# resero-labs/latok

Measured on NVIDIA B200. Metric: tokenized_text_throughput, higher is better.
Workload: dtype u8

## Files before the change

### latok_b200/csrc/latok_capi.cu

```cuda
#include "../../include/latok_b200.h"
#include "latok_internal.h"
#include "_gen/latok_tables.h"

#include <cstdarg>
#include <cstdio>
#include <cstdlib>
#include <cstring>
#include <new>
#include <vector>

using namespace latok;

namespace {

thread_local char g_err[512] = "";

int fail(int code, const char *fmt, ...)
{
    va_list ap;
    va_start(ap, fmt);
    vsnprintf(g_err, sizeof g_err, fmt, ap);
    va_end(ap);
    return code;
}
// ... 72 lines not shown
{
    if (na != nb) return false;
    std::vector<uint32_t> x(a, a + na), y(b, b + nb);
    for (auto v : x) {
        bool found = false;
        for (auto &w : y) if (w == v) { w = 0xFFFFFFFFu; found = true; break; }
        if (!found) return false;
    }
    return true;
}

}

struct Batch {
    DevBuf<uint8_t> d_in;
    DevBuf<long long> d_off, d_first, d_char_off, d_tok_off;
    DevBuf<int8_t> d_splits, d_feats, d_matrix;
    DevBuf<int32_t> d_spans;
    DevBuf<uint32_t> d_spans16;
    DevBuf<Result> d_result;
    PinBuf<Result> h_result;
    PinBuf<uint8_t> h_in;
    PinBuf<long long> h_off;
    cudaEvent_t ev_h2d = nullptr;
    cudaEvent_t ev_index = nullptr;
    cudaEvent_t ev_k0 = nullptr, ev_k1 = nullptr;
    cudaEvent_t ev_kdone = nullptr;
    bool submitted = false, sized = false, inputs_on_stream = false;
    const uint8_t *cur_in = nullptr;
    const long long *cur_off = nullptr;
    long long n_strings = 0, n_bytes = 0;
    uint32_t what = 0;
    long long n_chars = 0, n_tokens = 0, walks = 0;
    float kernel_ms = 0.f;
    void release()
    {
        d_in.release(); d_off.release(); d_first.release(); d_char_off.release(); d_tok_off.release();
        d_splits.release(); d_feats.release(); d_matrix.release(); d_spans.release(); d_spans16.release();
        d_result.release(); h_result.release(); h_in.release(); h_off.release();
        for (cudaEvent_t *ev : {&ev_h2d, &ev_index, &ev_k0, &ev_k1, &ev_kdone}) { if (*ev) cudaEventDestroy(*ev); *ev = nullptr; }
    }
};

struct latok_b200_engine {
    int device = 0;
    int n_sm = 0;
    cudaStream_t stream = nullptr, aux = nullptr, s_in = nullptr, s_out = nullptr;
    cudaEvent_t ev_t0 = nullptr, ev_t1 = nullptr, ev_b0 = nullptr, ev_b1 = nullptr;
    TableLayout tl{};
    RuleSet rules{};
    DevBuf<uint8_t> d_table, d_scratch, d_scratch2, d_scratch3;
    DevBuf<AggRec> agg;
    DevBuf<IncRec> inc;
    DevBuf<OpenSums> osum;
    DevBuf<uint32_t> d_planes;
    DevBuf<unsigned long long> span_scratch;
    DevBuf<long long> d_tok_bytes;
    DevBuf<unsigned> d_blk_local, d_group_tot;
    DevBuf<unsigned long long> d_group_pref;
    float last_token_bytes_ms = 0.f;
    unsigned epoch = 0;
    long long launches = 0;
    Batch set[2];
    int depth = 1;
    int q[2] = {0, 0}, nq = 0;
    int last = 1;
    Batch *front() { return nq ? &set[q[0]] : nullptr; }
};

extern "C" int latok_b200_set_error_(int code, const char *fmt, ...)
{
    va_list ap;
    va_start(ap, fmt);
    vsnprintf(g_err, sizeof g_err, fmt, ap);
    va_end(ap);
    return code;
// ... 103 lines not shown
        if (max_batch_bytes) {
            if (int r = b.d_in.ensure(max_batch_bytes + 64)) return r;
            if (int r = b.d_splits.ensure(max_batch_bytes + 64)) return r;
            if (int r = b.d_spans.ensure(2 * (max_batch_bytes / 3 + 1024))) return r;
        }
        if (max_strings) {
            if (int r = b.d_off.ensure((size_t)max_strings + 1)) return r;
            if (int r = b.d_char_off.ensure((size_t)max_strings + 1)) return r;
            if (int r = b.d_tok_off.ensure((size_t)max_strings + 1)) return r;
        }
        return 0;
    }();
    if (rc) { latok_b200_destroy(e); return rc; }
    *out = e;
    return LATOK_B200_OK;
}

int latok_b200_destroy(latok_b200_engine *e)
{
    if (!e) return LATOK_B200_OK;
    cudaSetDevice(e->device);
    for (cudaStream_t st : {e->stream, e->aux, e->s_in, e->s_out}) if (st) cudaStreamSynchronize(st);
    e->d_table.release(); e->d_scratch.release(); e->d_scratch2.release(); e->d_scratch3.release();
    e->agg.release(); e->inc.release(); e->osum.release(); e->d_planes.release(); e->span_scratch.release();
    e->d_tok_bytes.release(); e->d_blk_local.release(); e->d_group_tot.release(); e->d_group_pref.release();
    for (Batch &b : e->set) b.release();
    for (cudaEvent_t ev : {e->ev_t0, e->ev_t1, e->ev_b0, e->ev_b1}) if (ev) cudaEventDestroy(ev);
    for (cudaStream_t st : {e->stream, e->aux, e->s_in, e->s_out}) if (st) cudaStreamDestroy(st);
    delete e;
    return LATOK_B200_OK;
}

int latok_b200_set_pipeline_depth(latok_b200_engine *e, int depth)
{
    if (!e) return fail(LATOK_B200_EINVAL, "engine is NULL");
    if (depth != 1 && depth != 2) return fail(LATOK_B200_EINVAL, "pipeline depth must be 1 or 2");
    e->nq = 0;
    e->depth = depth;
    return LATOK_B200_OK;
}

int latok_b200_set_rules(latok_b200_engine *e, const int8_t *split, int sr, int sc, const int8_t *mask, int mr,
                         int mc, const int8_t *sym, int yr, int yc)
{
    if (!e) return fail(LATOK_B200_EINVAL, "engine is NULL");
    if (!split && !mask && !sym) { e->rules = default_rules(); return LATOK_B200_OK; }
    if (!split || !mask || !sym) return fail(LATOK_B200_EINVAL, "must specify split, mask and sym combo matrices");
// ... 23 lines not shown
    bool over = false;
    for (long long k = blockIdx.x * (long long)blockDim.x + threadIdx.x; k < n; k += (long long)gridDim.x * blockDim.x) {
        const int2 v = spans[k];
        over |= ((unsigned)v.x | (unsigned)v.y) > 0xFFFFu;
        out[k] = ((unsigned)v.x & 0xFFFFu) | ((unsigned)v.y << 16);
    }
    if (over) atomicOr(&res->error, 16u);
}

static int run_device(latok_b200_engine *e, Batch &b)
{
    const bool words = (b.what & LATOK_B200_MATRIX) != 0, feats = (b.what & LATOK_B200_FEATS) != 0;
    const bool use5 = !words && !getenv("LATOK_B200_FORCE_V4");
    bool shortg = b.n_bytes < 4096LL * (b.n_strings > 0 ? b.n_strings : 1);
    if (feats) shortg = false;
    if (const char *g = getenv("LATOK_B200_GEOMETRY")) shortg = g[0] == 's';
    const int range5 = shortg ? tokenize5_range_bytes_short() : tokenize5_range_bytes();
    const int nw5 = shortg ? tokenize5_ranges_per_tile_short() : tokenize5_ranges_per_tile();
    const int unit = use5 ? range5 : TILE;
    const long long nunits = b.n_bytes / unit + 1;
    const long long ntiles = use5 ? (nunits + nw5 - 1) / nw5 : nunits;
    const size_t plane_words = shortg ? tokenize5_plane_words_short(nunits) : tokenize5_plane_words(nunits);
    if (int r = b.d_first.ensure((size_t)nunits + 1)) return r;
    if ((size_t)ntiles > e->agg.cap) { CU(cudaStreamSynchronize(e->stream)); if (int r = e->agg.ensure((size_t)ntiles, true)) return r; }
    if ((size_t)ntiles > e->inc.cap) { CU(cudaStreamSynchronize(e->stream)); if (int r = e->inc.ensure((size_t)ntiles)) return r; }
    if (feats && (size_t)(use5 ? nunits : ntiles) > e->osum.cap) { CU(cudaStreamSynchronize(e->stream)); if (int r = e->osum.ensure((size_t)(use5 ? nunits : ntiles), true)) return r; }
    if (feats && use5 && plane_words > e->d_planes.cap) { CU(cudaStreamSynchronize(e->stream)); if (int r = e->d_planes.ensure(plane_words)) return r; }
    if (int r = b.d_splits.ensure((size_t)b.n_bytes + 64)) return r;
    if (int r = b.d_char_off.ensure((size_t)b.n_strings + 1)) return r;
    if (int r = b.d_tok_off.ensure((size_t)b.n_strings + 1)) return r;
    if (b.d_spans.cap < 2048) { if (int r = b.d_spans.ensure(2 * ((size_t)b.n_bytes / 3 + 1024))) return r; }
    if (b.what & LATOK_B200_FEATS) { if (int r = b.d_feats.ensure((b.d_spans.cap / 2) * NFEAT)) return r; }
    if (b.what & LATOK_B200_MATRIX) { if (int r = b.d_matrix.ensure(((size_t)b.n_bytes + 64) * NFEAT)) return r; }
    if (b.what & LATOK_B200_SPANS16) { if (int r = b.d_spans16.ensure(b.d_spans.cap / 2)) return r; }

    e->epoch = (e->epoch + 1) & 0x3FFFFFFFu;
    if (e->epoch == 0) {
        CU(cudaMemsetAsync(e->agg.p, 0, e->agg.cap * sizeof(AggRec), e->stream));
        e->epoch = 1;
    }
    Params p;
    memset(&p, 0, sizeof p);
    p.in = b.cur_in; p.n_bytes = b.n_bytes; p.offsets = b.cur_off; p.n_strings = b.n_strings;
    p.tile_first_str = b.d_first.p; p.ntiles = ntiles; p.nranges = nunits;
    p.splits = b.d_splits.p; p.char_off = b.d_char_off.p; p.spans = b.d_spans.p; p.tok_off = b.d_tok_off.p;
    p.feats = b.d_feats.p; p.matrix = b.d_matrix.p;
    p.cap_tokens = (long long)(b.d_spans.cap / 2);
    p.what = b.what & 15u;
    p.agg = e->agg.p; p.inc = e->inc.p; p.osum = e->osum.p; p.planes = e->d_planes.p; p.epoch = e->epoch;
    p.ticket = &b.d_result.p->ticket; p.ticket_base = 0;
    p.result = b.d_result.p;
    p.table_blob = e->d_table.p; p.tl = e->tl; p.rules = e->rules;
    int grid = e->n_sm * (!use5 ? tokenize_ctas_per_sm(e->tl, e->rules.is_default != 0, words, feats)
                          : shortg ? tokenize5_ctas_per_sm_short(e->tl, e->rules.is_default != 0, feats)
                                   : tokenize5_ctas_per_sm(e->tl, e->rules.is_default != 0, feats));
    if ((long long)grid > ntiles) grid = (int)ntiles;
    if (!use5) { if (int r = e->span_scratch.ensure((size_t)grid * 2 * SPAN_SCRATCH)) return r; }
    p.span_scratch = e->span_scratch.p;

    if (b.inputs_on_stream) CU(cudaStreamWaitEvent(e->aux, b.ev_h2d, 0));
    CU(cudaStreamWaitEvent(e->aux, b.ev_kdone, 0));
    CU(cudaMemsetAsync(b.d_result.p, 0, sizeof(Result), e->aux));
    CU(launch_tile_index(b.cur_off, b.n_strings, b.n_bytes, b.d_first.p, nunits, unit, b.d_result.p, e->aux));
    CU(cudaEventRecord(b.ev_index, e->aux));
    if (b.inputs_on_stream) CU(cudaStreamWaitEvent(e->stream, b.ev_h2d, 0));
    CU(cudaStreamWaitEvent(e->stream, b.ev_index, 0));
    CU(cudaEventRecord(b.ev_k0, e->stream));
    CU(!use5 ? launch_tokenize(p, grid, e->stream) : shortg ? launch_tokenize5_short(p, grid, e->stream) : launch_tokenize5(p, grid, e->stream));
    CU(cudaEventRecord(b.ev_k1, e->stream));
    e->launches += 2;
    if (b.what & LATOK_B200_SPANS16) {
        narrow_spans_kernel<<<e->n_sm * 8, 256, 0, e->stream>>>(reinterpret_cast<const int2 *>(b.d_spans.p), b.d_spans16.p, b.d_result.p, p.cap_tokens);
        CU(cudaGetLastError());
        e->launches += 1;
    }
    CU(cudaMemcpyAsync(b.h_result.p, b.d_result.p, sizeof(Result), cudaMemcpyDeviceToHost, e->stream));
    CU(cudaEventRecord(b.ev_kdone, e->stream));
    b.submitted = true;
    b.sized = false;
    return LATOK_B200_OK;
}

static int check_what(uint32_t &what)
{
    if (what & LATOK_B200_SPANS16) what |= LATOK_B200_SPANS;
    if (what == 0 || (what & ~31u)) return fail(LATOK_B200_EINVAL, "`what` must be a non-empty OR of LATOK_B200_SPLITS|SPANS|FEATS|MATRIX|SPANS16");
    return 0;
}

static int take_set(latok_b200_engine *e, Batch **out)
{
    if (e->depth == 1) e->nq = 0;
    if (e->nq >= e->depth) return fail(LATOK_B200_ESTATE, "%d batches are in flight: fetch and release the oldest one first", e->nq);
    const int s = e->last ^ 1;
    e->last = s;
    e->q[e->nq++] = s;
    *out = &e->set[s];
    return 0;
}
static void drop_last(latok_b200_engine *e) { if (e->nq) { --e->nq; e->last ^= 1; } }
// ... 75 lines not shown
    if (!b.submitted) return fail(LATOK_B200_ESTATE, "no batch submitted");
    for (int attempt = 0; attempt < 4 && !b.sized; ++attempt) {
        CU(cudaEventSynchronize(b.ev_kdone));
        const Result res = *b.h_result.p;
        if (res.error & 2u) { b.submitted = false; return fail(LATOK_B200_EINVAL, "offsets must start at 0, be non-decreasing and end at the buffer length"); }
        if (res.error & 1u) { b.submitted = false; return fail(LATOK_B200_EINTERNAL, "device look-back watchdog tripped"); }
        if (res.error & 8u) {
            b.submitted = false;
            return fail(LATOK_B200_EINTERNAL, "device consistency check failed: tile %llu G_in %llu K_in %llu n_own %lld ntok %lld c_lo %lld c_hi %lld",
                        res.prof[8], res.prof[9], res.prof[10], (long long)res.prof[11], (long long)res.prof[12], (long long)res.prof[13], (long long)res.prof[14]);
        }
        if ((res.error & 4u) || (long long)res.n_tokens > (long long)(b.d_spans.cap / 2)) {
            const size_t need = (size_t)res.n_tokens + 1024;
            if (int r = b.d_spans.ensure(2 * need)) return r;
            if (int r = run_device(e, b)) return r;
            continue;
        }
        if (res.error & 16u) { b.submitted = false; return fail(LATOK_B200_EINVAL, "LATOK_B200_SPANS16: a string of the batch has 65 536 or more characters"); }
        if (getenv("LATOK_B200_PRINT_PROF")) {
            fprintf(stderr, "[latok prof]");
            for (int i = 0; i < 16; ++i) fprintf(stderr, " %llu", res.prof[i]);
            fprintf(stderr, "\n");
        }
        b.n_chars = (long long)res.n_chars; b.n_tokens = (long long)res.n_tokens; b.walks = (long long)res.walks;
        float ms = 0.f;
        if (cudaEventElapsedTime(&ms, b.ev_k0, b.ev_k1) == cudaSuccess) b.kernel_ms = ms; else cudaGetLastError();
        b.sized = true;
    }
    if (!b.sized) return fail(LATOK_B200_EINTERNAL, "token capacity did not converge");
    return LATOK_B200_OK;
}

#define FRONT(e, b)                                                                  \
    if (!(e)) return fail(LATOK_B200_EINVAL, "engine is NULL");                      \
    if (!(e)->front()) return fail(LATOK_B200_ESTATE, "no batch submitted");         \
    if (int r_ = set_device(e)) return r_;                                           \
    Batch &b = *(e)->front()

int latok_b200_sizes(latok_b200_engine *e, int64_t *n_chars, int64_t *n_tokens)
{
    FRONT(e, b);
    if (int r = size_batch(e, b)) return r;
    if (n_chars) *n_chars = b.n_chars;
    if (n_tokens) *n_tokens = b.n_tokens;
    return LATOK_B200_OK;
}
// ... 211 lines not shown
```

### latok_b200/csrc/latok_device.cuh

```cuda
#pragma once
#include "latok_internal.h"
#include "latok_bits.h"

namespace latok {

constexpr uint32_t FIRSTBIT = 1u << 25;
constexpr uint32_t LASTBIT = 1u << 26;
constexpr uint32_t FEATMASK = (1u << NFEAT) - 1;
constexpr int NEG = -(1 << 28);
constexpr unsigned SPIN_LIMIT = 1u << 23;

__device__ __forceinline__ uint32_t mask_lt(int k) { return __funnelshift_lc(0xFFFFFFFFu, 0u, (unsigned)max(k, 0)); }
__device__ __forceinline__ uint32_t mask_lt_nn(int k) { return __funnelshift_lc(0xFFFFFFFFu, 0u, (unsigned)k); }
__device__ __forceinline__ uint32_t range_mask(int base, int lo, int hi)
{
    return mask_lt(hi - base) & ~mask_lt(lo - base);
}
__device__ __forceinline__ int widx(int c) { return 1 + c + ((c + 32) >> 5); }

struct Fn { int u, v; };
__device__ __forceinline__ Fn fn_id() { return Fn{0, NEG}; }
__device__ __forceinline__ Fn fn_compose(Fn f, Fn g)
{
    return Fn{max(f.u + g.u, NEG), max(max(f.v + g.u, g.v), NEG)};
// ... 25 lines not shown
                 "selp.u32 %0, 1, 0, P1;\n\t}" : "=r"(ok) : "r"(smem_u32(bar)), "r"(phase) : "memory");
    return ok != 0u;
}
__device__ __forceinline__ void mbar_wait(void *bar, uint32_t phase)
{
    while (!mbar_try_wait(bar, phase)) { }
}
__device__ __forceinline__ void tma_load_1d(void *dst, const void *src, uint32_t bytes, void *bar)
{
    asm volatile("cp.async.bulk.shared::cluster.global.mbarrier::complete_tx::bytes [%0], [%1], %2, [%3];"
                 ::"r"(smem_u32(dst)), "l"(src), "r"(bytes), "r"(smem_u32(bar)) : "memory");
}
__device__ __forceinline__ void fence_proxy_async() { asm volatile("fence.proxy.async.shared::cta;" ::: "memory"); }

__device__ __forceinline__ unsigned ld_volatile_u32(const unsigned *p)
{
    unsigned v;
    asm volatile("ld.volatile.global.u32 %0, [%1];" : "=r"(v) : "l"(p));
    return v;
}
__device__ __forceinline__ void st_volatile_u32(unsigned *p, unsigned v)
{
    asm volatile("st.volatile.global.u32 [%0], %1;" ::"l"(p), "r"(v) : "memory");
}

struct Tables {
    const uint16_t *ascii_feat;
    const uint16_t *class_feat;
    const latok_stage1_t *stage1;
    const uint8_t *stage2;
    uint32_t low_limit, high_first, high_last, high_feat;
};

__device__ __forceinline__ uint32_t class_of_cp(uint32_t cp, const Tables &t)
{
    if (cp < 0x80u) return t.ascii_feat[cp];
    if (cp < t.low_limit) {
        uint32_t blk = t.stage1[cp >> 7];
        uint32_t b = t.stage2[blk * 64u + ((cp & 127u) >> 1)];
        return t.class_feat[(cp & 1u) ? (b >> 4) : (b & 15u)];
    }
    return (cp >= t.high_first && cp <= t.high_last) ? t.high_feat : 0u;
}

template <class BytePtr>
__device__ __forceinline__ uint32_t classify_at(BytePtr p, const Tables &t)
// ... 353 lines not shown
```

### latok_b200/csrc/latok_internal.h

```cpp
#pragma once
#include "_gen/latok_table_types.h"
#include <cuda_runtime.h>
#include <stdint.h>

namespace latok {

constexpr int NT = 256;
constexpr int NWARP = NT / 32;
constexpr int LHALO = 32;
constexpr int WINB = NT * 32;
constexpr int RHALO = 224;
constexpr int TILE = WINB - LHALO - RHALO;
constexpr int TRUST_MARGIN = 12;
constexpr int FIRST_OWNED_THREAD = LHALO / 32;
constexpr int END_OWNED_THREAD = (LHALO + TILE) / 32;
constexpr int LUT_ENTRIES = 272;
constexpr int SPAN_STAGE = 1536;
constexpr int SPAN_SCRATCH = WINB + 64;

#ifndef LATOK_V5_RS
#define LATOK_V5_RS 4
#endif
#ifndef LATOK_V5_CTAS
#define LATOK_V5_CTAS 2
// ... 33 lines not shown
struct __align__(16) AggRec {
    unsigned status;
    unsigned n_lf;
    unsigned ntok_v;
    int u;
};
struct __align__(16) IncRec {
    unsigned long long G;
    unsigned long long base;
    unsigned long long K;
    int x;
    int pad;
};
struct __align__(16) OpenSums { unsigned has_split; unsigned pad[3]; unsigned sums[8]; };

struct Result {
    unsigned long long n_chars;
    unsigned long long n_tokens;
    unsigned long long walks;
    unsigned long long ticket;
    unsigned long long prof[16];
    unsigned int error;
    unsigned int abort_flag;
};

struct Params {
    const uint8_t *in;
    long long n_bytes;
    const long long *offsets;
    long long n_strings;
    const long long *tile_first_str;
    long long ntiles;
    long long nranges;
    int8_t *splits;
    long long *char_off;
    int32_t *spans;
    long long *tok_off;
    int8_t *feats;
    int8_t *matrix;
    long long cap_tokens;
    uint32_t what;
    AggRec *agg;
    IncRec *inc;
    OpenSums *osum;
    uint32_t *planes;
    void *span_scratch;
    unsigned epoch;
    unsigned long long *ticket;
    unsigned long long ticket_base;
    Result *result;
    const uint8_t *table_blob;
    TableLayout tl;
    RuleSet rules;
};

size_t tokenize_smem_bytes(const TableLayout &tl, bool want_words, bool want_feats);
int tokenize_ctas_per_sm(const TableLayout &tl, bool is_default, bool want_words, bool want_feats);
int tokenize5_range_bytes();
int tokenize5_ranges_per_tile();
int tokenize5_ctas_per_sm(const TableLayout &tl, bool is_default, bool want_feats);
size_t tokenize5_plane_words(long long nranges);
cudaError_t launch_tokenize5(const Params &p, int grid, cudaStream_t s);
int tokenize5_range_bytes_short();
int tokenize5_ranges_per_tile_short();
int tokenize5_ctas_per_sm_short(const TableLayout &tl, bool is_default, bool want_feats);
size_t tokenize5_plane_words_short(long long nranges);
cudaError_t launch_tokenize5_short(const Params &p, int grid, cudaStream_t s);
cudaError_t launch_tile_index(const long long *offsets, long long n_strings, long long n_bytes,
                              long long *tile_first_str, long long ntiles, int tile_bytes, Result *result, cudaStream_t s);
cudaError_t launch_tokenize(const Params &p, int grid, cudaStream_t s);
cudaError_t launch_block_mask(const int8_t *a1, long long s1, const int8_t *a2, long long s2, long long n,
                              int8_t *out, unsigned char *scratch, cudaStream_t s);
cudaError_t launch_combine_rows(const int8_t *m, long long m_rows, long long m_cols, long long stride_r,
                                long long stride_c, const int8_t *idx, int idx_rows, int idx_cols,
                                int8_t *out, cudaStream_t s);

long long token_bytes_words(long long n_bytes);
long long token_bytes_groups(long long n_bytes);
cudaError_t launch_token_bytes(const uint8_t *in, long long n_bytes, const long long *offsets, const long long *char_off,
                               const long long *tok_off, long long n_strings, long long n_tokens, const int32_t *spans,
                               long long *out, unsigned *word_local, unsigned *group_tot, unsigned long long *group_pref,
                               const uint8_t *table_blob, const TableLayout &tl, int n_sm, cudaStream_t s);

}
```

### latok_b200/csrc/latok_kernels.cu

```cuda
#include "latok_device.cuh"

namespace latok {

constexpr int VPAD = 256;
constexpr int NTS = 32;
constexpr int NTHREADS = NT + NTS;
constexpr int NBUF = 3;
enum { BAR_C = 1, BAR_AGG = 2, BAR_PRE = 4, BAR_LOADED = 6, BAR_FREE = 9 };

__device__ __forceinline__ int cbar_or(int pred)
{
    int r;
    asm volatile("{\n\t.reg .pred p, q;\n\tsetp.ne.s32 p, %1, 0;\n\tbar.red.or.pred q, 1, 256, p;\n\tselp.s32 %0, 1, 0, q;\n\t}" : "=r"(r) : "r"(pred) : "memory");
    return r;
}
#define CBAR() nb_sync(BAR_C, NT)

struct Slot {
    long long tile;
    int c_lo, c_hi, n_own, ntok, last_tile;
    int lft_rel;
    int v_tile;
    int nbf;
    int end0, end0_rel;
// ... 959 lines not shown
    if (is_default) {
        if (want_words) return want_feats ? ctas_one<true, true, true>(tl) : ctas_one<true, true, false>(tl);
        return want_feats ? ctas_one<true, false, true>(tl) : ctas_one<true, false, false>(tl);
    }
    if (want_words) return want_feats ? ctas_one<false, true, true>(tl) : ctas_one<false, true, false>(tl);
    return want_feats ? ctas_one<false, false, true>(tl) : ctas_one<false, false, false>(tl);
}

cudaError_t launch_tokenize(const Params &p, int grid, cudaStream_t s)
{
    const bool words = (p.what & 8u) != 0u, feats = (p.what & 4u) != 0u;
    if (p.rules.is_default) {
        if (words) return feats ? launch_one<true, true, true>(p, grid, s) : launch_one<true, true, false>(p, grid, s);
        return feats ? launch_one<true, false, true>(p, grid, s) : launch_one<true, false, false>(p, grid, s);
    }
    if (words) return feats ? launch_one<false, true, true>(p, grid, s) : launch_one<false, true, false>(p, grid, s);
    return feats ? launch_one<false, false, true>(p, grid, s) : launch_one<false, false, false>(p, grid, s);
}

__global__ void tile_index_kernel(const long long *offsets, long long n_strings, long long n_bytes,
                                  long long *first_str, long long ntiles, int TILE, Result *result)
{
    const long long s = blockIdx.x * (long long)blockDim.x + threadIdx.x;
    const int lane = threadIdx.x & 31;
    long long t_begin = 0, t_end = -1;
    if (s <= n_strings) {
        const long long cur = offsets[s];
        const long long prev = s ? offsets[s - 1] : -1;
        bool bad = cur < 0 || cur > n_bytes || cur < prev || (s == 0 && cur != 0) || (s == n_strings && cur != n_bytes);
        if (bad) atomicOr(&result->error, 2u);
        else {
            t_begin = prev < 0 ? 0 : prev / TILE + 1;
            t_end = cur / TILE;
            if (t_end > ntiles - 1) t_end = ntiles - 1;
        }
        if (s == n_strings) first_str[ntiles] = n_strings + 1;
    }
    const long long len = t_end - t_begin + 1;
    if (len > 0 && len <= 4)
        for (long long t = t_begin; t <= t_end; ++t) first_str[t] = s;
    unsigned long_mask = __ballot_sync(0xFFFFFFFFu, len > 4);
    while (long_mask) {
        const int src = __ffs(long_mask) - 1; long_mask &= long_mask - 1;
        const long long b = __shfl_sync(0xFFFFFFFFu, t_begin, src), e = __shfl_sync(0xFFFFFFFFu, t_end, src);
        const long long ss = __shfl_sync(0xFFFFFFFFu, s, src);
        for (long long t = b + lane; t <= e; t += 32) first_str[t] = ss;
    }
}

cudaError_t launch_tile_index(const long long *offsets, long long n_strings, long long n_bytes,
                              long long *tile_first_str, long long ntiles, int tile_bytes, Result *result, cudaStream_t s)
{
    const int bs = 256;
    const long long n = n_strings + 1;
    const unsigned grid = (unsigned)((n + bs - 1) / bs);
    tile_index_kernel<<<grid, bs, 0, s>>>(offsets, n_strings, n_bytes, tile_first_str, ntiles, tile_bytes, result);
    return cudaGetLastError();
}

constexpr int BM_NT = 1024;
__global__ void __launch_bounds__(BM_NT, 1)
block_mask_kernel(const int8_t *a1, long long s1, const int8_t *a2, long long s2, long long n, int8_t *out,
                  unsigned char *hot)
{
    __shared__ int scr[3 * 32 + 8];
    __shared__ int s_any_mark, s_any_space, s_carry;
    const int tid = threadIdx.x, lane = tid & 31, warp = tid >> 5;
    if (tid == 0) { s_any_mark = 0; s_any_space = 0; s_carry = 0; }
    __syncthreads();
    bool am = false, as = false;
// ... 116 lines not shown
```

### latok_b200/csrc/latok_tok5.cu

```cuda
#include "latok_device.cuh"

#ifdef LATOK_V5_SHORT
#define V5NS v5s
#define V5FN(name) name##_short
#else
#define V5NS v5
#define V5FN(name) name
#endif

namespace latok {
namespace V5NS {

constexpr int NW = V5_NW;
constexpr int NTH = (NW + 1) * 32;
constexpr int RS = V5_RS;
constexpr int STEP = 1024;
constexpr int WIN = RS * STEP;
constexpr int HALO = V5_HALO;
constexpr int HLANES = HALO / 32;
constexpr int RANGE = V5_RANGE;
constexpr int NMB = 7;
constexpr int MARGIN = 12;
constexpr int LPAD = 16;
constexpr int XBYTES = LPAD + WIN + 16;
constexpr int SSTAGE = 5 * 36 * 4;
constexpr int TCAP = 320;
constexpr int TSTAGE = (TCAP + 2) * 8;
constexpr int FLIST = 512;
constexpr int FSTAGE = 832;
constexpr int TWG = 12;
enum { BAR_AGG = 1, BAR_PRE = 3 };
static_assert(RANGE == WIN - HALO && HALO % 32 == 0 && RANGE % 16 == 0, "geometry");
static_assert(TSTAGE >= STEP + 64, "the token stage doubles as the byte stage of partly owned split-mask chunks");
static_assert(TSTAGE >= 1024 + FSTAGE && FSTAGE >= 15 + 32 * NFEAT + 8 && FSTAGE % 16 == 0, "token-feature mode: tails + row stage live in the token stage");

struct WAgg { int n_own, ntok, lft, v, flags, u, mb1, pad; };
struct Slot { unsigned long long G, K, base; int pad[2]; };
struct RInfo { int c_lo, c_hi, n_own, ntok, flags, pad[3]; };
struct Ctl {
    int tile_id[2], tk_cnt[2], tk_flag[2];
    int pad0[4];
    Slot slot[2];
    WAgg wagg[2][NW];
    RInfo rinfo[NW][2];
    int tokstep[NW][2][RS];
    int nsa[NW][2][RS];
};

struct Plan {
    int tables, ctl, mbar, sbm0, warp0, x[2], sst, tst, sbm, temp[2], per_warp, total;
};
__host__ __device__ inline Plan plan(const TableLayout &tl, bool is_default)
{
    Plan s; int o = 0;
    auto take = [&](int bytes) { int r = o; o += (bytes + 15) & ~15; return r; };
    s.tables = take(tl.stage2 - tl.lutv);
    s.ctl = take((int)sizeof(Ctl));
    s.mbar = take(8 * 2 * NW);
    s.sbm0 = take(RS * 32 * 4);
    s.warp0 = o;
    s.x[0] = take(XBYTES); s.x[1] = take(XBYTES);
    s.sst = take(SSTAGE);
    s.tst = take(TSTAGE);
    s.sbm = take(RS * 32 * 4);
    for (int b = 0; b < 2; ++b) s.temp[b] = is_default ? s.x[b] + LPAD : take(RS * TWG * 32 * 4);
    s.per_warp = o - s.warp0;
    s.total = s.warp0 + NW * s.per_warp;
    return s;
}

#ifdef LATOK_PROFILE
#define PROF5(i) do { if (lane == 0) { long long _t = clock64(); atomicAdd(&p.result->prof[i], (unsigned long long)(_t - _prof_t)); _prof_t = _t; } } while (0)
#else
#define PROF5(i) do { } while (0)
#endif

#ifndef LATOK_NO_HINTS
#define LIKELY(x) (__builtin_expect(!!(x), 1))
#define UNLIKELY(x) (__builtin_expect(!!(x), 0))
#else
#define LIKELY(x) (x)
#define UNLIKELY(x) (x)
#endif
constexpr unsigned FULL = 0xFFFFFFFFu;
constexpr int CINF = 0x3FFFFFFF;

__device__ __forceinline__ uint32_t pack_ncp(int n, int c0, int ps) { return (uint32_t)n | ((uint32_t)c0 << 6) | ((uint32_t)ps << 30); }
__device__ __forceinline__ int pk_n(uint32_t k) { return (int)(k & 63u); }
__device__ __forceinline__ int pk_c0(uint32_t k) { return (int)((k >> 6) & 8191u); }
__device__ __forceinline__ int pk_tp(uint32_t k) { return (int)((k >> 19) & 2047u); }
__device__ __forceinline__ uint32_t pk_ps(uint32_t k) { return (k >> 30) & 1u; }

__device__ __forceinline__ int bfind32(uint32_t x) { int r; asm("bfind.u32 %0, %1;" : "=r"(r) : "r"(x)); return r; }
__device__ __forceinline__ int ld_vs32(const int *p) { int v; asm volatile("ld.volatile.shared.s32 %0, [%1];" : "=r"(v) : "r"(smem_u32(p))); return v; }
__device__ __forceinline__ void st_vs32(int *p, int v) { asm volatile("st.volatile.shared.s32 [%0], %1;" ::"r"(smem_u32(p)), "r"(v) : "memory"); }

template <bool kDefault, bool kFeats>
__global__ void __launch_bounds__(NTH, kDefault ? LATOK_V5_CTAS : 1) tokenize5_kernel(const Params p)
{
    constexpr int NC = kDefault ? 3 : 4;
    constexpr int NY = kDefault ? 1 : 4;
    constexpr int NV = kDefault ? 3 : 5;
    constexpr int TWD = kDefault ? 8 : TWG;
    constexpr int I_S = kDefault ? 4 : 8, I_H = kDefault ? 5 : 9, I_F = kDefault ? 6 : 10, I_K = kDefault ? 7 : 11, I_E = kDefault ? 3 : 5;
    extern __shared__ __align__(128) unsigned char smem[];
    const Plan sp = plan(p.tl, kDefault);
    uint8_t *tableS = smem + sp.tables;
    Ctl &ctl = *reinterpret_cast<Ctl *>(smem + sp.ctl);
    unsigned long long *mbar = reinterpret_cast<unsigned long long *>(smem + sp.mbar);
    const int warp = threadIdx.x >> 5, lane = threadIdx.x & 31;
    const int cw = warp - 1;

    if (ld_volatile_u32(&p.result->error) & 2u) return;

    {
        const uint4 *src = reinterpret_cast<const uint4 *>(p.table_blob + p.tl.lutv);
        const int n16 = (p.tl.stage2 - p.tl.lutv) / 16;
        for (int i = threadIdx.x; i < n16; i += NTH) reinterpret_cast<uint4 *>(tableS)[i] = __ldg(src + i);
        if (threadIdx.x == 0) {
            for (int w = 0; w < 2 * NW; ++w) mbar_init(mbar + w, 1);
            for (int b = 0; b < 2; ++b) { ctl.tile_id[b] = 0; ctl.tk_cnt[b] = 0; ctl.tk_flag[b] = 0; }
        }
    }
    __syncthreads();
    const bool want_spans = (p.what & 2u) != 0u, want_splits = (p.what & 1u) != 0u;
    const int ntiles_i = (int)p.ntiles;

    Tables tb;
    tb.ascii_feat = reinterpret_cast<const uint16_t *>(tableS + (p.tl.ascii_feat - p.tl.lutv));
    tb.class_feat = reinterpret_cast<const uint16_t *>(tableS + (p.tl.class_feat - p.tl.lutv));
    tb.stage1 = reinterpret_cast<const latok_stage1_t *>(tableS + (p.tl.stage1 - p.tl.lutv));
    tb.stage2 = p.table_blob + p.tl.stage2;
    tb.low_limit = p.tl.low_limit; tb.high_first = p.tl.high_first; tb.high_last = p.tl.high_last; tb.high_feat = p.tl.high_feat;

    int tw = cw;
    auto wbase_of = [&]() -> unsigned char * { return smem + sp.warp0 + tw * sp.per_warp; };
    unsigned char *wbase = smem + sp.warp0 + (cw < 0 ? 0 : cw) * sp.per_warp;
    uint8_t *sst = wbase + (sp.sst - sp.warp0);
    int2 *tst = reinterpret_cast<int2 *>(wbase + (sp.tst - sp.warp0));
    auto Xof = [&](int b) -> uint8_t * { return wbase_of() + (sp.x[b] - sp.warp0); };
    auto sbm_of = [&]() -> uint32_t * {
        return reinterpret_cast<uint32_t *>(warp == 0 ? smem + sp.sbm0 : wbase_of() + (sp.sbm - sp.warp0));
    };
    auto tempof = [&](int b) -> uint32_t * { return reinterpret_cast<uint32_t *>(wbase_of() + (sp.temp[b] - sp.warp0)); };
    auto SA = [&](uint32_t *base, int js, int ln) -> uint32_t * { return kDefault ? base + js * 256 + ln * 4 : base + (js * 32 + ln) * TWD; };
    auto SW = [&](int w) -> int { return kDefault ? (w < 4 ? w : 124 + w) : w; };
    const uint32_t *lutv = reinterpret_cast<const uint32_t *>(tableS);
// ... 630 lines not shown
#endif
            }
            if (lane == 0) {
                IncRec *ir = p.inc + tile;
                uint4 a, bq;
                const unsigned long long Gn = pre.G + (unsigned long long)n, Kn = pre.K + (unsigned long long)ntok;
                const unsigned long long Bn = lft_rel >= 0 ? pre.G + (unsigned long long)lft_rel : pre.base;
                a.x = (unsigned)Gn; a.y = (unsigned)(Gn >> 32); a.z = (unsigned)Bn; a.w = (unsigned)(Bn >> 32);
                bq.x = (unsigned)Kn; bq.y = (unsigned)(Kn >> 32); bq.z = (unsigned)v; bq.w = 0;
                st_rec(ir, a); st_rec(reinterpret_cast<uint4 *>(ir) + 1, bq);
                __threadfence();
                uint4 r;
                r.x = (p.epoch << 2) | 2u;
                r.y = (unsigned)n | ((lft_rel >= 0 ? (unsigned)(lft_rel + 1) : 0u) << 16);
                r.z = (unsigned)ntok | ((unsigned)v << 16); r.w = 0;
                st_rec(p.agg + tile, r);
                Slot &sl = ctl.slot[s];
                sl.G = pre.G; sl.K = pre.K; sl.base = pre.base;
                __threadfence_block();
            }
            __syncwarp();
            nb_arrive(BAR_PRE + s, NTH);
        }
        return;
    }

    auto output = [&](const long long r, const int buf, unsigned long long G_in, unsigned long long K_in, unsigned long long base_in) {
        const RInfo ri = ctl.rinfo[cw][buf];
        const bool have = (ri.flags & 1) != 0, closed = (ri.flags & 2) != 0, lo_found = (ri.flags & 4) != 0, last_range = (ri.flags & 8) != 0;
        if (!have) return;
        const int c_lo = ri.c_lo, c_hi = ri.c_hi, n_own = ri.n_own, ntok_range = ri.ntok;
        const long long w0 = r * (long long)RANGE;
        const long long rem64 = p.n_bytes - w0;
        const int nb_win = rem64 > (long long)(WIN + 64) ? WIN + 64 : (int)rem64;
        const uint32_t *tempS = tempof(buf);
        if (K_in + (unsigned long long)ntok_range > (unsigned long long)p.cap_tokens && lane == 0) atomicOr(&p.result->error, 4u);
        if (G_in + (unsigned long long)n_own > (unsigned long long)p.n_bytes || K_in + (unsigned long long)ntok_range > (unsigned long long)p.n_bytes + 1ull) {
            if (lane == 0 && atomicOr(&p.result->error, 8u) == 0u) {
                p.result->prof[8] = (unsigned long long)r; p.result->prof[9] = G_in; p.result->prof[10] = K_in;
                p.result->prof[11] = (unsigned long long)(long long)n_own; p.result->prof[12] = (unsigned long long)(long long)ntok_range;
                p.result->prof[13] = (unsigned long long)(long long)c_lo; p.result->prof[14] = (unsigned long long)(long long)c_hi;
            }
            return;
        }
        int cur_base = c_lo - (int)(long long)(G_in - base_in);
        int ktok = 0;
// ... 420 lines not shown
            if (lane == 0) {
                uint4 *o = reinterpret_cast<uint4 *>(p.osum + r);
                st_rec(o + 1, make_uint4(fc[0], fc[1], fc[2], fc[3]));
                st_rec(o + 2, make_uint4(fc[4], fc[5], fc[6], 0u));
                __threadfence();
                st_rec(o, make_uint4(fc_hit ? 1u : 0u, p.epoch, 0u, 0u));
            }
        }
        if (last_range && lane == 0) {
            p.result->n_chars = G_in + (unsigned long long)n_own;
            p.result->n_tokens = K_in + (unsigned long long)ntok_range;
        }
    };

    auto next_tile = [&](int k) -> int {
        const int s = k & 1;
        int t = 0;
        if (lane == 0) {
            const int old = atomicAdd(&ctl.tk_cnt[s], 1);
            if (old == NW - 1) st_vs32(&ctl.tk_cnt[s], 0);
            if (old == 0) {
                const unsigned long long tk = atomicAdd(p.ticket, 1ull) - p.ticket_base;
                t = tk < (unsigned long long)ntiles_i ? (int)tk : ntiles_i;
                st_vs32(&ctl.tile_id[s], t);
                __threadfence_block();
                st_vs32(&ctl.tk_flag[s], k + 1);
            } else {
                unsigned spins = 0;
                while (ld_vs32(&ctl.tk_flag[s]) != k + 1) { if (++spins > (1u << 26)) { atomicOr(&p.result->error, 1u); break; } }
                t = ld_vs32(&ctl.tile_id[s]);
            }
        }
        return __shfl_sync(FULL, t, 0);
    };
    auto post = [&](int s) {
        if (lane == 0) {
            WAgg &a = ctl.wagg[s][cw];
            a.n_own = a_n_own; a.ntok = a_ntok; a.lft = a_lft; a.v = a_v; a.flags = a_flags; a.u = a_u; a.mb1 = a_mb1;
            __threadfence_block();
        }
        __syncwarp();
        nb_arrive(BAR_AGG + s, NTH);
    };
    auto wait_window = [&](int b, unsigned &phase_bits) {
        unsigned spins = 0;
        while (!mbar_try_wait(mbar + 2 * cw + b, (phase_bits >> b) & 1u)) {
// ... 32 lines not shown
    bool pending[2] = {false, false};
    int tile_cur = next_tile(0), tile_prev = -1;
    if (tile_cur < ntiles_i) pending[0] = begin_load((long long)tile_cur * NW + cw, 0);
    for (int k = 0;; ++k) {
        const int s = k & 1;
        if (tile_cur < ntiles_i) {
            build_map((long long)tile_cur * NW + cw);
            if (s == 0 ? pending[0] : pending[1]) wait_window(s, phase_bits);
            __syncwarp();
            PROF5(0);
            analyze((long long)tile_cur * NW + cw, s, 0, -1);
            post(s);
        } else {
            nb_arrive(BAR_AGG + s, NTH);
        }
        if (tile_prev >= 0) finish_tile(tile_prev, k - 1);
        if (tile_cur >= ntiles_i) break;
        const int tile_next = next_tile(k + 1);
        bool pn = false;
        if (tile_next < ntiles_i) pn = begin_load((long long)tile_next * NW + cw, s ^ 1);
        if (s == 0) pending[1] = pn; else pending[0] = pn;
        tile_prev = tile_cur; tile_cur = tile_next;
    }
}

template <bool kDefault, bool kFeats>
static cudaError_t launch_one(const Params &p, int grid, cudaStream_t s)
{
    const size_t smem = (size_t)plan(p.tl, kDefault).total;
    static size_t configured = 0;
    if (configured < smem) {
        cudaError_t e = cudaFuncSetAttribute(tokenize5_kernel<kDefault, kFeats>, cudaFuncAttributeMaxDynamicSharedMemorySize, (int)smem);
        if (e != cudaSuccess) return e;
        configured = smem;
    }
    tokenize5_kernel<kDefault, kFeats><<<grid, NTH, smem, s>>>(p);
    return cudaGetLastError();
}

template <bool kDefault, bool kFeats>
static int ctas_one(const TableLayout &tl)
{
    int nb = 0;
    const size_t smem = (size_t)plan(tl, kDefault).total;
    cudaFuncSetAttribute(tokenize5_kernel<kDefault, kFeats>, cudaFuncAttributeMaxDynamicSharedMemorySize, (int)smem);
    if (cudaOccupancyMaxActiveBlocksPerMultiprocessor(&nb, tokenize5_kernel<kDefault, kFeats>, NTH, smem) != cudaSuccess) { cudaGetLastError(); return 1; }
    return nb < 1 ? 1 : nb;
}

}

int V5FN(tokenize5_range_bytes)() { return V5NS::RANGE; }
int V5FN(tokenize5_ranges_per_tile)() { return V5NS::NW; }
size_t V5FN(tokenize5_plane_words)(long long nranges) { return (size_t)nranges * V5NS::RS * NFEAT * 32; }

int V5FN(tokenize5_ctas_per_sm)(const TableLayout &tl, bool is_default, bool want_feats)
{
    if (is_default) return want_feats ? V5NS::ctas_one<true, true>(tl) : V5NS::ctas_one<true, false>(tl);
    return want_feats ? V5NS::ctas_one<false, true>(tl) : V5NS::ctas_one<false, false>(tl);
}

cudaError_t V5FN(launch_tokenize5)(const Params &p, int grid, cudaStream_t s)
{
    const bool feats = (p.what & 4u) != 0u;
    if (p.rules.is_default) return feats ? V5NS::launch_one<true, true>(p, grid, s) : V5NS::launch_one<true, false>(p, grid, s);
    return feats ? V5NS::launch_one<false, true>(p, grid, s) : V5NS::launch_one<false, false>(p, grid, s);
}

}
```

Measured before the change: 430.1.

## Fuse tile-index pass and result reset into tokenize5 kernel with PDL launch

```diff
diff --git a/latok_b200/csrc/latok_capi.cu b/latok_b200/csrc/latok_capi.cu
--- a/latok_b200/csrc/latok_capi.cu
+++ b/latok_b200/csrc/latok_capi.cu
@@ -118,6 +118,9 @@
     PinBuf<Result> h_result;
     PinBuf<uint8_t> h_in;
     PinBuf<long long> h_off;
+    DevBuf<AggRec> agg;
+    DevBuf<IncRec> inc;
+    unsigned long long chunk_base = 0, done_base = 0;
     cudaEvent_t ev_h2d = nullptr;
     cudaEvent_t ev_index = nullptr;
     cudaEvent_t ev_k0 = nullptr, ev_k1 = nullptr;
@@ -129,12 +132,19 @@
     uint32_t what = 0;
     long long n_chars = 0, n_tokens = 0, walks = 0;
     float kernel_ms = 0.f;
+#ifdef LATOK_PROFILE
+    DevBuf<unsigned long long> d_tl;
+    int tl_grid = 0; unsigned tl_epoch = 0;
+#endif
     void release()
     {
         d_in.release(); d_off.release(); d_first.release(); d_char_off.release(); d_tok_off.release();
         d_splits.release(); d_feats.release(); d_matrix.release(); d_spans.release(); d_spans16.release();
-        d_result.release(); h_result.release(); h_in.release(); h_off.release();
+        d_result.release(); h_result.release(); h_in.release(); h_off.release(); agg.release(); inc.release();
         for (cudaEvent_t *ev : {&ev_h2d, &ev_index, &ev_k0, &ev_k1, &ev_kdone}) { if (*ev) cudaEventDestroy(*ev); *ev = nullptr; }
+#ifdef LATOK_PROFILE
+        d_tl.release();
+#endif
     }
 };
 
@@ -146,8 +156,6 @@
     TableLayout tl{};
     RuleSet rules{};
     DevBuf<uint8_t> d_table, d_scratch, d_scratch2, d_scratch3;
-    DevBuf<AggRec> agg;
-    DevBuf<IncRec> inc;
     DevBuf<OpenSums> osum;
     DevBuf<uint32_t> d_planes;
     DevBuf<unsigned long long> span_scratch;
@@ -297,7 +305,7 @@
     cudaSetDevice(e->device);
     for (cudaStream_t st : {e->stream, e->aux, e->s_in, e->s_out}) if (st) cudaStreamSynchronize(st);
     e->d_table.release(); e->d_scratch.release(); e->d_scratch2.release(); e->d_scratch3.release();
-    e->agg.release(); e->inc.release(); e->osum.release(); e->d_planes.release(); e->span_scratch.release();
+    e->osum.release(); e->d_planes.release(); e->span_scratch.release();
     e->d_tok_bytes.release(); e->d_blk_local.release(); e->d_group_tot.release(); e->d_group_pref.release();
     for (Batch &b : e->set) b.release();
     for (cudaEvent_t ev : {e->ev_t0, e->ev_t1, e->ev_b0, e->ev_b1}) if (ev) cudaEventDestroy(ev);
@@ -367,8 +375,8 @@
     const long long ntiles = use5 ? (nunits + nw5 - 1) / nw5 : nunits;
     const size_t plane_words = shortg ? tokenize5_plane_words_short(nunits) : tokenize5_plane_words(nunits);
     if (int r = b.d_first.ensure((size_t)nunits + 1)) return r;
-    if ((size_t)ntiles > e->agg.cap) { CU(cudaStreamSynchronize(e->stream)); if (int r = e->agg.ensure((size_t)ntiles, true)) return r; }
-    if ((size_t)ntiles > e->inc.cap) { CU(cudaStreamSynchronize(e->stream)); if (int r = e->inc.ensure((size_t)ntiles)) return r; }
+    if ((size_t)ntiles > b.agg.cap) { CU(cudaStreamSynchronize(e->stream)); if (int r = b.agg.ensure((size_t)ntiles, true)) return r; }
+    if ((size_t)ntiles > b.inc.cap) { CU(cudaStreamSynchronize(e->stream)); if (int r = b.inc.ensure((size_t)ntiles)) return r; }
     if (feats && (size_t)(use5 ? nunits : ntiles) > e->osum.cap) { CU(cudaStreamSynchronize(e->stream)); if (int r = e->osum.ensure((size_t)(use5 ? nunits : ntiles), true)) return r; }
     if (feats && use5 && plane_words > e->d_planes.cap) { CU(cudaStreamSynchronize(e->stream)); if (int r = e->d_planes.ensure(plane_words)) return r; }
     if (int r = b.d_splits.ensure((size_t)b.n_bytes + 64)) return r;
@@ -381,7 +389,7 @@
 
     e->epoch = (e->epoch + 1) & 0x3FFFFFFFu;
     if (e->epoch == 0) {
-        CU(cudaMemsetAsync(e->agg.p, 0, e->agg.cap * sizeof(AggRec), e->stream));
+        for (Batch &x : e->set) if (x.agg.p) CU(cudaMemsetAsync(x.agg.p, 0, x.agg.cap * sizeof(AggRec), e->stream));
         e->epoch = 1;
     }
     Params p;
@@ -392,7 +400,7 @@
     p.feats = b.d_feats.p; p.matrix = b.d_matrix.p;
     p.cap_tokens = (long long)(b.d_spans.cap / 2);
     p.what = b.what & 15u;
-    p.agg = e->agg.p; p.inc = e->inc.p; p.osum = e->osum.p; p.planes = e->d_planes.p; p.epoch = e->epoch;
+    p.agg = b.agg.p; p.inc = b.inc.p; p.osum = e->osum.p; p.planes = e->d_planes.p; p.epoch = e->epoch;
     p.ticket = &b.d_result.p->ticket; p.ticket_base = 0;
     p.result = b.d_result.p;
     p.table_blob = e->d_table.p; p.tl = e->tl; p.rules = e->rules;
@@ -402,25 +410,47 @@
     if ((long long)grid > ntiles) grid = (int)ntiles;
     if (!use5) { if (int r = e->span_scratch.ensure((size_t)grid * 2 * SPAN_SCRATCH)) return r; }
     p.span_scratch = e->span_scratch.p;
-
-    if (b.inputs_on_stream) CU(cudaStreamWaitEvent(e->aux, b.ev_h2d, 0));
-    CU(cudaStreamWaitEvent(e->aux, b.ev_kdone, 0));
-    CU(cudaMemsetAsync(b.d_result.p, 0, sizeof(Result), e->aux));
-    CU(launch_tile_index(b.cur_off, b.n_strings, b.n_bytes, b.d_first.p, nunits, unit, b.d_result.p, e->aux));
-    CU(cudaEventRecord(b.ev_index, e->aux));
-    if (b.inputs_on_stream) CU(cudaStreamWaitEvent(e->stream, b.ev_h2d, 0));
-    CU(cudaStreamWaitEvent(e->stream, b.ev_index, 0));
-    CU(cudaEventRecord(b.ev_k0, e->stream));
-    CU(!use5 ? launch_tokenize(p, grid, e->stream) : shortg ? launch_tokenize5_short(p, grid, e->stream) : launch_tokenize5(p, grid, e->stream));
-    CU(cudaEventRecord(b.ev_k1, e->stream));
-    e->launches += 2;
+#ifdef LATOK_PROFILE
+    if (use5 && getenv("LATOK_B200_TIMELINE") && grid <= TL_MAX_CTAS) {
+        if (int r = b.d_tl.ensure((size_t)TL_MAX_CTAS * TL_SLOTS)) return r;
+        p.timeline = b.d_tl.p; b.tl_grid = grid; b.tl_epoch = e->epoch;
+    }
+#endif
+
+    if (!use5) {
+        if (b.inputs_on_stream) CU(cudaStreamWaitEvent(e->aux, b.ev_h2d, 0));
+        CU(cudaStreamWaitEvent(e->aux, b.ev_kdone, 0));
+        CU(cudaMemsetAsync(b.d_result.p, 0, sizeof(Result), e->aux));
+        b.chunk_base = b.done_base = 0;
+        CU(launch_tile_index(b.cur_off, b.n_strings, b.n_bytes, b.d_first.p, nunits, unit, b.d_result.p, e->aux));
+        CU(cudaEventRecord(b.ev_index, e->aux));
+        if (b.inputs_on_stream) CU(cudaStreamWaitEvent(e->stream, b.ev_h2d, 0));
+        CU(cudaStreamWaitEvent(e->stream, b.ev_index, 0));
+        CU(cudaEventRecord(b.ev_k0, e->stream));
+        CU(launch_tokenize(p, grid, e->stream));
+        CU(cudaEventRecord(b.ev_k1, e->stream));
+        e->launches += 2;
+    } else {
+        p.chunk_base = b.chunk_base; p.done_base = b.done_base;
+        if (b.inputs_on_stream) CU(cudaStreamWaitEvent(e->stream, b.ev_h2d, 0));
+        CU(cudaEventRecord(b.ev_k0, e->stream));
+        CU(shortg ? launch_tokenize5_short(p, grid, e->stream) : launch_tokenize5(p, grid, e->stream));
+        CU(cudaEventRecord(b.ev_k1, e->stream));
+        const long long chunks = (b.n_strings + (shortg ? tokenize5_index_chunk_short() : tokenize5_index_chunk())) /
+                                 (shortg ? tokenize5_index_chunk_short() : tokenize5_index_chunk());
+        b.chunk_base += (unsigned long long)(chunks + grid);
+        b.done_base += (unsigned long long)chunks;
+        e->launches += 1;
+    }
     if (b.what & LATOK_B200_SPANS16) {
         narrow_spans_kernel<<<e->n_sm * 8, 256, 0, e->stream>>>(reinterpret_cast<const int2 *>(b.d_spans.p), b.d_spans16.p, b.d_result.p, p.cap_tokens);
         CU(cudaGetLastError());
         e->launches += 1;
     }
-    CU(cudaMemcpyAsync(b.h_result.p, b.d_result.p, sizeof(Result), cudaMemcpyDeviceToHost, e->stream));
-    CU(cudaEventRecord(b.ev_kdone, e->stream));
+    CU(cudaEventRecord(b.ev_index, e->stream));
+    CU(cudaStreamWaitEvent(e->aux, b.ev_index, 0));
+    CU(cudaMemcpyAsync(b.h_result.p, b.d_result.p, sizeof(Result), cudaMemcpyDeviceToHost, e->aux));
+    CU(cudaEventRecord(b.ev_kdone, e->aux));
     b.submitted = true;
     b.sized = false;
     return LATOK_B200_OK;
@@ -542,6 +572,26 @@
             for (int i = 0; i < 16; ++i) fprintf(stderr, " %llu", res.prof[i]);
             fprintf(stderr, "\n");
         }
+#ifdef LATOK_PROFILE
+        if (const char *path = getenv("LATOK_B200_TIMELINE")) {
+            if (FILE *f = fopen(path, "a")) {
+                for (Batch &x : e->set) {
+                    if (!x.tl_grid) continue;
+                    std::vector<unsigned long long> h((size_t)x.tl_grid * TL_SLOTS);
+                    CU(cudaMemcpy(h.data(), x.d_tl.p, h.size() * sizeof(unsigned long long), cudaMemcpyDeviceToHost));
+                    fprintf(f, "{\"epoch\": %u, \"grid\": %d, \"cta\": [", x.tl_epoch, x.tl_grid);
+                    for (int c = 0; c < x.tl_grid; ++c) {
+                        fprintf(f, "%s[", c ? ", " : "");
+                        for (int k = 0; k < TL_SLOTS; ++k) fprintf(f, "%s%llu", k ? ", " : "", h[(size_t)c * TL_SLOTS + k]);
+                        fprintf(f, "]");
+                    }
+                    fprintf(f, "]}\n");
+                    x.tl_grid = 0;
+                }
+                fclose(f);
+            }
+        }
+#endif
         b.n_chars = (long long)res.n_chars; b.n_tokens = (long long)res.n_tokens; b.walks = (long long)res.walks;
         float ms = 0.f;
         if (cudaEventElapsedTime(&ms, b.ev_k0, b.ev_k1) == cudaSuccess) b.kernel_ms = ms; else cudaGetLastError();
diff --git a/latok_b200/csrc/latok_device.cuh b/latok_b200/csrc/latok_device.cuh
--- a/latok_b200/csrc/latok_device.cuh
+++ b/latok_b200/csrc/latok_device.cuh
@@ -71,6 +71,52 @@
 __device__ __forceinline__ void st_volatile_u32(unsigned *p, unsigned v)
 {
     asm volatile("st.volatile.global.u32 [%0], %1;" ::"l"(p), "r"(v) : "memory");
+}
+__device__ __forceinline__ unsigned ld_acquire_u32(const unsigned *p)
+{
+    unsigned v;
+    asm volatile("ld.acquire.gpu.global.u32 %0, [%1];" : "=r"(v) : "l"(p) : "memory");
+    return v;
+}
+__device__ __forceinline__ unsigned long long ld_acquire_u64(const unsigned long long *p)
+{
+    unsigned long long v;
+    asm volatile("ld.acquire.gpu.global.u64 %0, [%1];" : "=l"(v) : "l"(p) : "memory");
+    return v;
+}
+__device__ __forceinline__ void st_release_u32(unsigned *p, unsigned v)
+{
+    asm volatile("st.release.gpu.global.u32 [%0], %1;" ::"l"(p), "r"(v) : "memory");
+}
+__device__ __forceinline__ void grid_dep_wait() { asm volatile("griddepcontrol.wait;" ::: "memory"); }
+__device__ __forceinline__ void grid_dep_launch_dependents() { asm volatile("griddepcontrol.launch_dependents;" ::: "memory"); }
+
+__device__ __forceinline__ bool index_string(long long s, long long cur, long long prev, const long long n_strings,
+                                             const long long n_bytes, long long *first_str, const long long ntiles, const int unit)
+{
+    const int lane = threadIdx.x & 31;
+    long long t_begin = 0, t_end = -1;
+    bool ok = true;
+    if (s <= n_strings) {
+        ok = !(cur < 0 || cur > n_bytes || cur < prev || (s == 0 && cur != 0) || (s == n_strings && cur != n_bytes));
+        if (ok) {
+            t_begin = prev < 0 ? 0 : prev / unit + 1;
+            t_end = cur / unit;
+            if (t_end > ntiles - 1) t_end = ntiles - 1;
+        }
+        if (s == n_strings) first_str[ntiles] = n_strings + 1;
+    }
+    const long long len = t_end - t_begin + 1;
+    if (len > 0 && len <= 4)
+        for (long long t = t_begin; t <= t_end; ++t) first_str[t] = s;
+    unsigned long_mask = __ballot_sync(0xFFFFFFFFu, len > 4);
+    while (long_mask) {
+        const int src = __ffs(long_mask) - 1; long_mask &= long_mask - 1;
+        const long long b = __shfl_sync(0xFFFFFFFFu, t_begin, src), e = __shfl_sync(0xFFFFFFFFu, t_end, src);
+        const long long ss = __shfl_sync(0xFFFFFFFFu, s, src);
+        for (long long t = b + lane; t <= e; t += 32) first_str[t] = ss;
+    }
+    return ok;
 }
 
 struct Tables {
diff --git a/latok_b200/csrc/latok_internal.h b/latok_b200/csrc/latok_internal.h
--- a/latok_b200/csrc/latok_internal.h
+++ b/latok_b200/csrc/latok_internal.h
@@ -79,7 +79,13 @@
     unsigned long long prof[16];
     unsigned int error;
     unsigned int abort_flag;
+    unsigned long long chunk, chunk_done;
+    unsigned int gen;
+    unsigned int pad;
 };
+
+enum { TL_START, TL_INDEX, TL_FIRST, TL_PAST_END, TL_EXIT, TL_SLOTS };
+constexpr int TL_MAX_CTAS = 1024;
 
 struct Params {
     const uint8_t *in;
@@ -105,7 +111,9 @@
     unsigned epoch;
     unsigned long long *ticket;
     unsigned long long ticket_base;
+    unsigned long long chunk_base, done_base;
     Result *result;
+    unsigned long long *timeline;
     const uint8_t *table_blob;
     TableLayout tl;
     RuleSet rules;
@@ -115,11 +123,13 @@
 int tokenize_ctas_per_sm(const TableLayout &tl, bool is_default, bool want_words, bool want_feats);
 int tokenize5_range_bytes();
 int tokenize5_ranges_per_tile();
+int tokenize5_index_chunk();
 int tokenize5_ctas_per_sm(const TableLayout &tl, bool is_default, bool want_feats);
 size_t tokenize5_plane_words(long long nranges);
 cudaError_t launch_tokenize5(const Params &p, int grid, cudaStream_t s);
 int tokenize5_range_bytes_short();
 int tokenize5_ranges_per_tile_short();
+int tokenize5_index_chunk_short();
 int tokenize5_ctas_per_sm_short(const TableLayout &tl, bool is_default, bool want_feats);
 size_t tokenize5_plane_words_short(long long nranges);
 cudaError_t launch_tokenize5_short(const Params &p, int grid, cudaStream_t s);
diff --git a/latok_b200/csrc/latok_kernels.cu b/latok_b200/csrc/latok_kernels.cu
--- a/latok_b200/csrc/latok_kernels.cu
+++ b/latok_b200/csrc/latok_kernels.cu
@@ -1005,30 +1005,9 @@
                                   long long *first_str, long long ntiles, int TILE, Result *result)
 {
     const long long s = blockIdx.x * (long long)blockDim.x + threadIdx.x;
-    const int lane = threadIdx.x & 31;
-    long long t_begin = 0, t_end = -1;
-    if (s <= n_strings) {
-        const long long cur = offsets[s];
-        const long long prev = s ? offsets[s - 1] : -1;
-        bool bad = cur < 0 || cur > n_bytes || cur < prev || (s == 0 && cur != 0) || (s == n_strings && cur != n_bytes);
-        if (bad) atomicOr(&result->error, 2u);
-        else {
-            t_begin = prev < 0 ? 0 : prev / TILE + 1;
-            t_end = cur / TILE;
-            if (t_end > ntiles - 1) t_end = ntiles - 1;
-        }
-        if (s == n_strings) first_str[ntiles] = n_strings + 1;
-    }
-    const long long len = t_end - t_begin + 1;
-    if (len > 0 && len <= 4)
-        for (long long t = t_begin; t <= t_end; ++t) first_str[t] = s;
-    unsigned long_mask = __ballot_sync(0xFFFFFFFFu, len > 4);
-    while (long_mask) {
-        const int src = __ffs(long_mask) - 1; long_mask &= long_mask - 1;
-        const long long b = __shfl_sync(0xFFFFFFFFu, t_begin, src), e = __shfl_sync(0xFFFFFFFFu, t_end, src);
-        const long long ss = __shfl_sync(0xFFFFFFFFu, s, src);
-        for (long long t = b + lane; t <= e; t += 32) first_str[t] = ss;
-    }
+    long long cur = 0, prev = -1;
+    if (s <= n_strings) { cur = offsets[s]; prev = s ? offsets[s - 1] : -1; }
+    if (!index_string(s, cur, prev, n_strings, n_bytes, first_str, ntiles, TILE)) atomicOr(&result->error, 2u);
 }
 
 cudaError_t launch_tile_index(const long long *offsets, long long n_strings, long long n_bytes,
diff --git a/latok_b200/csrc/latok_tok5.cu b/latok_b200/csrc/latok_tok5.cu
--- a/latok_b200/csrc/latok_tok5.cu
+++ b/latok_b200/csrc/latok_tok5.cu
@@ -29,6 +29,8 @@
 constexpr int FLIST = 512;
 constexpr int FSTAGE = 832;
 constexpr int TWG = 12;
+constexpr int IX_PER = 8;
+constexpr int IX_CHUNK = NTH * IX_PER;
 enum { BAR_AGG = 1, BAR_PRE = 3 };
 static_assert(RANGE == WIN - HALO && HALO % 32 == 0 && RANGE % 16 == 0, "geometry");
 static_assert(TSTAGE >= STEP + 64, "the token stage doubles as the byte stage of partly owned split-mask chunks");
@@ -39,7 +41,8 @@
 struct RInfo { int c_lo, c_hi, n_own, ntok, flags, pad[3]; };
 struct Ctl {
     int tile_id[2], tk_cnt[2], tk_flag[2];
-    int pad0[4];
+    int ix_chunk;
+    int pad0[3];
     Slot slot[2];
     WAgg wagg[2][NW];
     RInfo rinfo[NW][2];
@@ -71,8 +74,13 @@
 
 #ifdef LATOK_PROFILE
 #define PROF5(i) do { if (lane == 0) { long long _t = clock64(); atomicAdd(&p.result->prof[i], (unsigned long long)(_t - _prof_t)); _prof_t = _t; } } while (0)
+__device__ __forceinline__ unsigned long long gtimer() { unsigned long long t; asm volatile("mov.u64 %0, %%globaltimer;" : "=l"(t)); return t; }
+#define TL5(slot) do { if (p.timeline) p.timeline[(size_t)blockIdx.x * TL_SLOTS + (slot)] = gtimer(); } while (0)
+#define TL5_EXIT() do { if (p.timeline && lane == 0) atomicMax(&p.timeline[(size_t)blockIdx.x * TL_SLOTS + TL_EXIT], gtimer()); } while (0)
 #else
 #define PROF5(i) do { } while (0)
+#define TL5(slot) do { } while (0)
+#define TL5_EXIT() do { } while (0)
 #endif
 
 #ifndef LATOK_NO_HINTS
@@ -111,18 +119,70 @@
     const int warp = threadIdx.x >> 5, lane = threadIdx.x & 31;
     const int cw = warp - 1;
 
-    if (ld_volatile_u32(&p.result->error) & 2u) return;
-
+    if (kFeats) grid_dep_wait();
+    if (threadIdx.x == 0) TL5(TL_START);
+
+    const long long nchunks = (p.n_strings + IX_CHUNK) / IX_CHUNK;
     {
+        for (;;) {
+            if (threadIdx.x == 0) {
+                const unsigned long long c = atomicAdd(&p.result->chunk, 1ull) - p.chunk_base;
+                if (c == 0) {
+                    Result *r = p.result;
+                    r->n_chars = 0; r->n_tokens = 0; r->walks = 0; r->ticket = 0; r->error = 0; r->abort_flag = 0;
+                    for (int i = 0; i < 16; ++i) r->prof[i] = 0;
+                    __threadfence();
+                    st_release_u32(&r->gen, p.epoch);
+                }
+                ctl.ix_chunk = c < (unsigned long long)nchunks ? (int)c : (int)nchunks;
+            }
+            __syncthreads();
+            const long long c = ctl.ix_chunk;
+            if (c >= nchunks) break;
+            const long long s0 = c * IX_CHUNK + (long long)threadIdx.x * IX_PER;
+            long long o[IX_PER + 1];
+#pragma unroll
+            for (int j = 0; j <= IX_PER; ++j) {
+                const long long s = s0 - 1 + j;
+                o[j] = s >= 0 && s <= p.n_strings ? p.offsets[s] : -1;
+            }
+            bool ok = true;
+#pragma unroll
+            for (int j = 0; j < IX_PER; ++j)
+                ok &= index_string(s0 + j, o[j + 1], o[j], p.n_strings, p.n_bytes, const_cast<long long *>(p.tile_first_str), p.nranges, RANGE);
+            if (!ok) {
+                unsigned spins = 0;
+                while (ld_acquire_u32(&p.result->gen) != p.epoch && ++spins < (1u << 26)) { }
+                atomicOr(&p.result->error, 2u);
+            }
+            __threadfence();
+            __syncthreads();
+            if (threadIdx.x == 0) atomicAdd(&p.result->chunk_done, 1ull);
+        }
+    }
+
+    {
+#ifdef LATOK_PROFILE
+        if (threadIdx.x == 0 && p.timeline) p.timeline[(size_t)blockIdx.x * TL_SLOTS + TL_EXIT] = 0;
+#endif
         const uint4 *src = reinterpret_cast<const uint4 *>(p.table_blob + p.tl.lutv);
         const int n16 = (p.tl.stage2 - p.tl.lutv) / 16;
         for (int i = threadIdx.x; i < n16; i += NTH) reinterpret_cast<uint4 *>(tableS)[i] = __ldg(src + i);
         if (threadIdx.x == 0) {
             for (int w = 0; w < 2 * NW; ++w) mbar_init(mbar + w, 1);
             for (int b = 0; b < 2; ++b) { ctl.tile_id[b] = 0; ctl.tk_cnt[b] = 0; ctl.tk_flag[b] = 0; }
+            unsigned spins = 0;
+            while (ld_acquire_u64(&p.result->chunk_done) - p.done_base < (unsigned long long)nchunks) {
+                if (++spins > (1u << 26)) { atomicOr(&p.result->error, 1u); break; }
+            }
+            TL5(TL_INDEX);
         }
     }
     __syncthreads();
+    if (ld_volatile_u32(&p.result->error) & 2u) {
+        grid_dep_wait();
+        return;
+    }
     const bool want_spans = (p.what & 2u) != 0u, want_splits = (p.what & 1u) != 0u;
     const int ntiles_i = (int)p.ntiles;
 
@@ -799,6 +859,7 @@
             __syncwarp();
             nb_arrive(BAR_PRE + s, NTH);
         }
+        TL5_EXIT();
         return;
     }
 
@@ -1265,6 +1326,12 @@
             if (old == 0) {
                 const unsigned long long tk = atomicAdd(p.ticket, 1ull) - p.ticket_base;
                 t = tk < (unsigned long long)ntiles_i ? (int)tk : ntiles_i;
+                if (k == 0) TL5(TL_FIRST);
+                if (t == ntiles_i) {
+                    TL5(TL_PAST_END);
+                    grid_dep_wait();
+                    grid_dep_launch_dependents();
+                }
                 st_vs32(&ctl.tile_id[s], t);
                 __threadfence_block();
                 st_vs32(&ctl.tk_flag[s], k + 1);
@@ -1343,6 +1410,7 @@
         if (s == 0) pending[1] = pn; else pending[0] = pn;
         tile_prev = tile_cur; tile_cur = tile_next;
     }
+    TL5_EXIT();
 }
 
 template <bool kDefault, bool kFeats>
@@ -1355,8 +1423,13 @@
         if (e != cudaSuccess) return e;
         configured = smem;
     }
-    tokenize5_kernel<kDefault, kFeats><<<grid, NTH, smem, s>>>(p);
-    return cudaGetLastError();
+    cudaLaunchAttribute attr;
+    attr.id = cudaLaunchAttributeProgrammaticStreamSerialization;
+    attr.val.programmaticStreamSerializationAllowed = 1;
+    cudaLaunchConfig_t cfg = {};
+    cfg.gridDim = dim3((unsigned)grid); cfg.blockDim = dim3(NTH); cfg.dynamicSmemBytes = smem; cfg.stream = s;
+    cfg.attrs = &attr; cfg.numAttrs = 1;
+    return cudaLaunchKernelEx(&cfg, tokenize5_kernel<kDefault, kFeats>, p);
 }
 
 template <bool kDefault, bool kFeats>
@@ -1373,6 +1446,7 @@
 
 int V5FN(tokenize5_range_bytes)() { return V5NS::RANGE; }
 int V5FN(tokenize5_ranges_per_tile)() { return V5NS::NW; }
+int V5FN(tokenize5_index_chunk)() { return V5NS::IX_CHUNK; }
 size_t V5FN(tokenize5_plane_words)(long long nranges) { return (size_t)nranges * V5NS::RS * NFEAT * 32; }
 
 int V5FN(tokenize5_ctas_per_sm)(const TableLayout &tl, bool is_default, bool want_feats)
```

After: 427.4 (median of 6 runs). About the same (-0.6%).
